# hsiehScalAR/KNODE-Cosserat

Measured on AMD Instinct MI355X. Metric: rod-steps/sec (N=100 segments, batch=1024), higher is better.
Workload: dtype f64

## Files before the change

knode-cosserat_amd/csrc/kr_mso_impl.hpp:

```cpp
#pragma once
#include "kr_ms_impl.hpp"

namespace kr {

constexpr int MSO_B0 = 7 + 17 * (MS_P - 1);
#ifndef KR_MSO_LAG
#define KR_MSO_LAG 1
#endif
constexpr int MSO_LAG = KR_MSO_LAG;
static_assert(MSO_B0 + MS_P <= WAVE, "the verifying lanes must fit beside the forward-difference lanes");

template <typename T, int HS>
__host__ __device__ inline size_t mso_lds_elems(int N) {
  return ms_lds_elems<T, HS>(N, true, false) + 80;
}

__device__ __forceinline__ void wave_sync_lds() {
  __builtin_amdgcn_fence(__ATOMIC_ACQ_REL, "wavefront");
  __builtin_amdgcn_wave_barrier();
}

#define KR_LDS __attribute__((address_space(3)))
template <typename T, int NV>
__device__ __forceinline__ void lds_load_vec(const T* src, T (&v)[NV]) {
  using V = typename Vec16<T>::type;
  constexpr int n = Vec16<T>::n;
  static_assert(NV % n == 0, "vector load needs a multiple of 16 bytes");
  const KR_LDS V* s = (const KR_LDS V*)src;
#pragma unroll
  for (int c = 0; c < NV / n; ++c) {
    const V x = s[c];
#pragma unroll
    for (int e = 0; e < n; ++e) v[c * n + e] = x[e];
  }
}
template <typename T, int NV>
__device__ __forceinline__ void lds_store_vec(T* dst, const T (&v)[NV]) {
  using V = typename Vec16<T>::type;
  constexpr int n = Vec16<T>::n;
  static_assert(NV % n == 0, "vector store needs a multiple of 16 bytes");
  KR_LDS V* d = (KR_LDS V*)dst;
#pragma unroll
  for (int c = 0; c < NV / n; ++c) {
    V x;
#pragma unroll
    for (int e = 0; e < n; ++e) x[e] = v[c * n + e];
    d[c] = x;
  }
}

#ifdef KR_MS_STAMPS
struct MsoStats { unsigned long long total = 0, sweeps = 0, merged = 0, quick = 0, chord = 0, rejects = 0, retries = 0, rebuilds = 0, t_sweep = 0, t_alg = 0, t_pred = 0, t_verdict = 0, t_cond = 0, t_fin = 0, t_upd = 0, t_v1 = 0, t_v2 = 0, t_c1 = 0, t_c2 = 0, t_copy = 0; };
#endif

template <typename T, bool DIAG, int HS, int OCC = 1, typename PSRC = RodConst<T>>
__global__ __launch_bounds__(WAVE * MS_WPB, OCC) void mso_sim_kernel(const PSRC Pa, const SimArgs<T> A) {
  extern __shared__ __attribute__((aligned(16))) unsigned char smem_raw[];
  const int N = rod_src_N<T>(Pa);
  const int lane = threadIdx.x & (WAVE - 1);
  const int wv = threadIdx.x / WAVE;
  const int64_t rod = (int64_t)blockIdx.x * MS_WPB + wv;
  if (rod >= A.B) return;
  const auto& Pc = rod_src_row<T>(Pa, rod);
  const size_t rod_elems = (size_t)N * KR_SLOTS;
  const int64_t T_steps = A.T_steps;
  const MsLds<T> L = ms_carve<T, HS>(reinterpret_cast<T*>(smem_raw) + (size_t)wv * mso_lds_elems<T, HS>(N), N, true, false);
  T* const Xs = L.Xs;
  T* const Es = L.Es;
  T* const XB = L.XB;
  T* const Tm = L.Tm;
  T* const XsB = L.c12 + (size_t)N * 12;
  T* const EsB = Es + MSO_B0 * MS_YP;
  const MsRole R = ms_role(lane, N);
  const int iv = R.iv, col = R.col;
  const bool isA = lane < MSO_B0;
  const bool isB = lane >= MSO_B0 && lane < MSO_B0 + MS_P;
  const int ib = isB ? lane - MSO_B0 : 0;
  const int s_l = isB ? ms_interval_start(ib, R.sbase, R.srem) : R.s_i;
  const int len_l = isB ? R.sbase + (ib < R.srem ? 1 : 0) : R.len_i;
  ms_cold_fill<T>(rod_src_mem<T>(Pa, rod), L.cold, lane);
  wave_sync();

  auto state_ptr = [&](int64_t k) -> T* { return A.states + (A.ring ? k % 3 : k) * A.slot_elems + rod * rod_elems; };
  T* const lead0 = L.c12;
  const ptrdiff_t lead_d = L.hist - L.c12;
  auto lead_of = [&](int64_t t) -> T* { return lead0 + (ptrdiff_t)(t & 1) * lead_d; };
  auto rebuild = [&](int64_t t) {
    const T* cur = state_ptr(t);
    const T* prv = t > 0 ? state_ptr(t - 1) : (A.prev_init ? A.prev_init + rod * rod_elems : cur);
    T* const lc = lead_of(t);
    T* const lp = lead_of(t - 1);
    for (int j = lane; j < N; j += WAVE) {
      T cv[12], pv[12];
      load_hist_vec<T, 12>(cur + (size_t)j * KR_SLOTS, cv);
      load_hist_vec<T, 12>(prv + (size_t)j * KR_SLOTS, pv);
      lds_store_vec<T, 12>(lc + (size_t)j * 12, cv);
      lds_store_vec<T, 12>(lp + (size_t)j * 12, pv);
    }
    wave_sync();
  };
  const T* ctl = A.ctl + rod * T_steps * 4;
  auto load_fc = [&](int64_t t) -> V3<T> {
    V3<T> tf{T(0), T(0), T(0)};
#pragma unroll
    for (int k = 0; k < 4; ++k) {
      const T tt = ctl[t * 4 + k];
      tf.x += tt * L.cold[CD_TDIRS + k * 3 + 0];
      tf.y += tt * L.cold[CD_TDIRS + k * 3 + 1];
      tf.z += tt * L.cold[CD_TDIRS + k * 3 + 2];
    }
    return {L.cold[CD_RHOAG] + tf.x, L.cold[CD_RHOAG + 1] + tf.y, L.cold[CD_RHOAG + 2] + tf.z};
  };

  const T* s0 = state_ptr(0);
  const T* sp0 = A.prev_init ? A.prev_init + rod * rod_elems : s0;
  MsPred<T> Q;
  double* img = A.pred_io ? A.pred_io + (size_t)rod * MS_PRED_ROWS * WAVE : nullptr;
  if (img && A.pred_load) ms_pred_load<T>(Q, img, lane);
  else ms_pred_init<T>(Q, lane, R, s0, sp0, A.prev_init != nullptr, A.predictor);
  V3<T> vlast, ulast;
  {
    const T* cl = s0 + (size_t)(N - 1) * KR_SLOTS;
    vlast = {cl[SL_V], cl[SL_V + 1], cl[SL_V + 2]};
    ulast = {cl[SL_U], cl[SL_U + 1], cl[SL_U + 2]};
  }
  const T tol = A.tol, tolA = A.tolA, fd_eps = A.fd_eps;
  const int maxit = A.maxit;
  T kappa = Q.kappa;
  T Gguess = lane < 6 ? A.G[rod * 6 + lane] : T(0);
  MsStamps stamps;
#ifdef KR_MS_STAMPS
  MsoStats st;
  unsigned long long t_begin, tq;
  KR_STAMP(t_begin);
  tq = t_begin;
#endif

  rebuild(0);

  int64_t tA = 0;
  bool merged = false;
  int it = 0;
  int order = Q.next_order;
  bool retried = false;
  T dn_prev = T(-1);
  bool have_fac = false, below = false;
  float amp = -1.f;
  T dnB = T(-1);
  float ampB = -1.f;
  bool belowB = false;
  int itB = 0, orderB = 0;
  bool pred_skip = false;
  bool reverify = false;
  int64_t resume_at = T_steps;
  T Xreg[MS_P - 1][2];
#pragma unroll
  for (int g = 0; g < MS_P - 1; ++g) Xreg[g][0] = Xreg[g][1] = T(0);
  const int kp = lane & 3;
  const int r = 3 + (lane >> 2);
  const bool plane = lane < 3 * (MS_P - 1);
  const int pi = plane ? lane / 3 : 0;
  const int prow = plane ? lane - 3 * pi : 0;
  const bool glane = lane >= WAVE - 6;
  V3<T> fcA = load_fc(0), fcB = fcA;
  V3<T> fcN = load_fc(T_steps > 1 ? 1 : 0);
  static_assert(DIAG, "the in-sweep history record assumes diagonal material matrices");
  T hk_a[3], hk_b[3], hk_c[3];
#pragma unroll
  for (int c = 0; c < 3; ++c) {
    hk_a[c] = L.cold[CD_KSEI + 4 * c] * L.cold[CD_KSEV + c];
    hk_b[c] = -L.cold[CD_KSEI + 4 * c] * L.cold[CD_BSE + 4 * c];
    hk_c[c] = -L.cold[CD_KBTI + 4 * c] * L.cold[CD_BBT + 4 * c];
  }

  ms_pred_guess<T>(Q, order, lane, L.cold, Xs);
  wave_sync_lds();
  if (order <= 0 && lane < 6) Xs[0 * MS_YP + 7 + lane] = Gguess;
  wave_sync_lds();

  struct Upd { T updP, updG, xsP, xsG, xsY[MS_P - 1]; };

  while (true) {
    const bool runA = tA < T_steps;
    const int64_t tB = tA - 1;
    T yr[19];
    {
      const T* src = isB ? XsB + ib * MS_YP : Xs + iv * MS_YP;
#pragma unroll
      for (int q = 0; q < 19; ++q) yr[q] = src[q];
    }
    const T hstep = (isA && col > 0) ? fd_eps * fmax(fabs(Xs[iv * MS_YP + (R.comp > 0 ? R.comp : 3)]), T(1)) : T(1);
#pragma unroll
    for (int q = 3; q < 19; ++q) yr[q] += (isA && q == R.comp) ? hstep : T(0);
    RodState<T> y = rows_to_state(yr);
    const V3<T> fc = isB ? fcB : fcA;
    const int lag = (isA && merged) ? MSO_LAG : 0;
    const bool act = isB ? merged : (isA && runA);
    const int trips = R.lmax + ((merged && runA) ? MSO_LAG : 0);
    T* const out_rod = state_ptr(tB + 1);
    auto point_of = [&](int k) -> int {
      const int kk = k - lag;
      return s_l + (kk < 0 ? 0 : (kk < len_l ? kk : len_l - 1));
    };
    const T* const lead_n = lead_of(isB ? tB : tA);
    const T* const lead_o = lead_of(isB ? tB + 1 : tB);
    auto hist_form = [&](const T (&la)[12], const T (&lb)[12]) __attribute__((always_inline)) -> RodHist<T> {
      T raw[12];
#pragma unroll
      for (int c = 0; c < 12; ++c) raw[c] = A.hc1 * la[c] + A.hc2 * lb[c];
      RodHist<T> h;
      h.qh = {raw[0], raw[1], raw[2]};
      h.wh = {raw[3], raw[4], raw[5]};
      h.vh = {raw[6], raw[7], raw[8]};
      h.uh = {raw[9], raw[10], raw[11]};
      h.av = {hk_b[0] * raw[6] + hk_a[0], hk_b[1] * raw[7] + hk_a[1], hk_b[2] * raw[8] + hk_a[2]};
      h.au = {hk_c[0] * raw[9], hk_c[1] * raw[10], hk_c[2] * raw[11]};
      return h;
    };
    auto hist_at = [&](int j) __attribute__((always_inline)) -> RodHist<T> {
      T la[12], lb[12];
      lds_load_vec<T, 12>(lead_n + (size_t)j * 12, la);
      lds_load_vec<T, 12>(lead_o + (size_t)j * 12, lb);
      return hist_form(la, lb);
    };
    RodHist<T> hst = hist_at(point_of(0));
    if (!merged) {
      auto fd_point = [&](int j, T dsl) __attribute__((always_inline)) {
        RodState<T> k1;
        V3<T> v, u;
        ode_eval<T, DIAG>(Pc, y, hst, fc, k1, v, u);
        hst = hist_at(j + 1);
        y = state_axpy(y, dsl, k1);
      };
#pragma unroll 2
      for (int t = 0; t < R.sbase; ++t) fd_point(R.s_i + t, Pc.ds);
      if (R.srem) fd_point(R.s_i + (R.len_i > R.sbase ? R.sbase : R.sbase - 1), R.len_i > R.sbase ? Pc.ds : T(0));
    } else {
      const bool lean = A.ring && tB + 4 <= T_steps;
      T* const lead_w = lead_of(tB + 1);
      auto trip = [&](int k, auto full_tag) __attribute__((always_inline)) {
        constexpr bool FULL = decltype(full_tag)::value;
        const int kk = k - lag;
        const bool live = FULL ? act : (act && kk >= 0 && kk < len_l);
        const int j = FULL ? s_l + kk : point_of(k);
        T la[12], lb[12];
        if constexpr (MSO_LAG >= 2) {
          const int jn = FULL ? j + 1 : point_of(k + 1);
          lds_load_vec<T, 12>(lead_n + (size_t)jn * 12, la);
          lds_load_vec<T, 12>(lead_o + (size_t)jn * 12, lb);
        }
        RodState<T> k1;
        V3<T> v, u;
        ode_eval<T, DIAG>(Pc, y, hst, fc, k1, v, u);
        if constexpr (MSO_LAG >= 2) {
          hst = hist_form(la, lb);
          asm volatile("" : "+v"(hst.qh.x), "+v"(hst.qh.y), "+v"(hst.qh.z), "+v"(hst.wh.x), "+v"(hst.wh.y), "+v"(hst.wh.z));
          asm volatile("" : "+v"(hst.vh.x), "+v"(hst.vh.y), "+v"(hst.vh.z), "+v"(hst.uh.x), "+v"(hst.uh.y), "+v"(hst.uh.z));
          asm volatile("" : "+v"(hst.av.x), "+v"(hst.av.y), "+v"(hst.av.z), "+v"(hst.au.x), "+v"(hst.au.y), "+v"(hst.au.z));
        }
        if (isB && live) {
          T rec[KR_SLOTS];
          record_from(y, v, u, rec);
          T lead[12];
#pragma unroll
          for (int c = 0; c < 12; ++c) lead[c] = rec[c];
          if constexpr (FULL) {
            if (!lean) {
              T rest[KR_SLOTS - 12];
#pragma unroll
              for (int c = 0; c < KR_SLOTS - 12; ++c) rest[c] = rec[12 + c];
              store_vec<T, KR_SLOTS - 12>(out_rod + (size_t)j * KR_SLOTS + 12, rest);
            }
          } else {
            store_record(out_rod + (size_t)j * KR_SLOTS, rec);
          }
          lds_store_vec<T, 12>(lead_w + (size_t)j * 12, lead);
        }
        if constexpr (MSO_LAG < 2) hst = hist_at(FULL ? j + 1 : point_of(k + 1));
        const T dsl = live ? Pc.ds : T(0);
        y = state_axpy(y, dsl, k1);
      };
      int k = 0;
      for (; k < MSO_LAG && k < trips; ++k) trip(k, std::false_type{});
#pragma unroll 2
      for (; k < R.sbase; ++k) trip(k, std::true_type{});
      for (; k < trips; ++k) trip(k, std::false_type{});
    }
#ifdef KR_MS_STAMPS
    KR_STAMP_ADD(st.t_sweep, tq);
    st.sweeps += 1;
    if (merged) st.merged += 1;
#endif

    T er[19];
    state_to_rows(y, er);
    T d[6];
    T updY[MS_P - 1];
    T* dYb = XB;
    float dnf = 0.f;
    bool finite = true;
    Upd U;

    auto finish = [&](const T* X, auto base_slot) -> float {
      T* sp = Tm;
      if (kp == 0) {
#pragma unroll
        for (int g = 1; g < MS_P - 1; ++g) dYb[g * MS_YP + r] = updY[g - 1];
      }
      wave_sync_lds();
      if (plane) {
        const int l0 = pi == 0 ? 0 : 7 + 17 * (pi - 1);
        T s = Es[base_slot(pi) * MS_YP + prow] - X[(pi + 1) * MS_YP + prow];
        T av[16], dv[16];
#pragma unroll
        for (int c = 0; c < 16; ++c) {
          const bool use = pi > 0 || c < 6;
          av[c] = use ? Es[(l0 + 1 + c) * MS_YP + prow] : T(0);
          dv[c] = pi > 0 ? dYb[pi * MS_YP + 3 + c] : T(0);
        }
        __builtin_amdgcn_sched_barrier(0);
        T s2 = T(0);
#pragma unroll
        for (int c = 0; c < 16; c += 2) {
          const T da = pi > 0 ? dv[c] : (c < 6 ? d[c < 6 ? c : 0] : T(0));
          const T db = pi > 0 ? dv[c + 1] : (c + 1 < 6 ? d[c + 1 < 6 ? c + 1 : 0] : T(0));
          s = fma(av[c], da, s);
          s2 = fma(av[c + 1], db, s2);
        }
        sp[pi * 3 + prow] = s + s2;
      }
      wave_sync_lds();
      float nf = 0.f;
      U.updP = T(0); U.updG = T(0); U.xsP = T(0); U.xsG = T(0);
      if (plane) {
        U.xsP = X[(pi + 1) * MS_YP + prow];
#pragma unroll
        for (int i = 0; i < MS_P - 1; ++i) {
          const T t = sp[i * 3 + prow];
          U.updP += i <= pi ? t : T(0);
        }
        nf = update_ratio(U.updP, U.xsP);
      }
      if (glane) {
        const int k = lane - (WAVE - 6);
        U.xsG = X[0 * MS_YP + 7 + k];
        U.updG = k == 0 ? d[0] : k == 1 ? d[1] : k == 2 ? d[2] : k == 3 ? d[3] : k == 4 ? d[4] : d[5];
        nf = fmaxf(nf, update_ratio(U.updG, U.xsG));
      }
#pragma unroll
      for (int g = 1; g < MS_P; ++g) {
        U.xsY[g - 1] = T(0);
        if (((g - 1) & 3) == kp) {
          U.xsY[g - 1] = X[g * MS_YP + r];
          nf = fmaxf(nf, update_ratio(updY[g - 1], U.xsY[g - 1]));
        }
      }
      return wave_max_nonneg(nf);
    };
    auto apply = [&](T* X) {
      if (plane) X[(pi + 1) * MS_YP + prow] = U.xsP + U.updP;
      if (glane) X[0 * MS_YP + 7 + (lane - (WAVE - 6))] = U.xsG + U.updG;
#pragma unroll
      for (int g = 1; g < MS_P; ++g)
        if (((g - 1) & 3) == kp) X[g * MS_YP + r] = U.xsY[g - 1] + updY[g - 1];
    };

    if (merged) {
      if (isB) {
#pragma unroll
        for (int q = 0; q < 19; ++q) EsB[ib * MS_YP + q] = er[q];
        if (ib == MS_P - 1) {
          T rec[KR_SLOTS];
          record_from(y, vlast, ulast, rec);
          store_record(out_rod + (size_t)(N - 1) * KR_SLOTS, rec);
          T lead[12];
#pragma unroll
          for (int c = 0; c < 12; ++c) lead[c] = rec[c];
          lds_store_vec<T, 12>(lead_of(tB + 1) + (size_t)(N - 1) * 12, lead);
          if (A.tip) {
            T* tp = A.tip + (rod * T_steps + tB) * 3;
            tp[0] = y.p.x; tp[1] = y.p.y; tp[2] = y.p.z;
          }
        }
      }
      wave_sync_lds();
#ifdef KR_MS_STAMPS
      unsigned long long tv;
      { KR_STAMP(tv); st.t_v1 += tv - tq; }
#endif
      float rn = 0.f;
      if (lane < 3 * MS_YP) {
        const int g = lane / MS_YP, q = lane - MS_YP * g;
        const T x = XsB[(g + 1) * MS_YP + q];
        rn = update_ratio(EsB[g * MS_YP + q] - x, x);
      } else if (lane < 3 * MS_YP + 6) {
        const int k = lane - 3 * MS_YP;
        const T e = EsB[(MS_P - 1) * MS_YP + 7 + k];
        rn = update_ratio(L.cold[CD_FTIP + k] - e, e);
      }
      rn = wave_max_nonneg(rn);
#ifdef KR_MS_STAMPS
      KR_STAMP_ADD(st.t_v2, tv);
#endif
      const float est = ampB * rn;
      bool accepted = A.residual_test != 0 && ampB > 0.f && T(256) * (T)est <= tol;
      float dnv = est;
#ifdef KR_MS_STAMPS
      if (accepted) st.quick += 1;
#endif
      if (!accepted) {
        T* ach = XB;
        T* rt = XB + 4 * MS_YP;
        dYb = XB + MS_YP * 8;
        T areg[MS_P - 1];
        areg[0] = EsB[0 * MS_YP + r] - XsB[1 * MS_YP + r];
        if (kp == 0) ach[1 * MS_YP + r] = areg[0];
        wave_sync_lds();
#pragma unroll
        for (int g = 1; g < MS_P; ++g) {
          const int l0 = 7 + 17 * (g - 1);
          T av[4], xv[4];
#pragma unroll
          for (int cc = 0; cc < 4; ++cc) {
            av[cc] = Es[(l0 + 1 + 4 * kp + cc) * MS_YP + r];
            xv[cc] = ach[g * MS_YP + 3 + 4 * kp + cc];
          }
          const T e0 = EsB[g * MS_YP + r];
          const T ynext = g < MS_P - 1 ? XsB[(g + 1) * MS_YP + r] : T(0);
          T part = fma(av[0], xv[0], av[1] * xv[1]) + fma(av[2], xv[2], av[3] * xv[3]);
          part += quad_xor<0xB1>(part);
          part += quad_xor<0x4E>(part);
          if (g < MS_P - 1) {
            areg[g] = e0 - ynext + part;
            if (kp == 0) ach[(g + 1) * MS_YP + r] = areg[g];
          } else if (kp == 0 && r >= 7 && r < 13) {
            rt[r - 7] = L.cold[CD_FTIP + (r - 7)] - e0 - part;
          }
          wave_sync_lds();
        }
        {
          T rtv[6];
#pragma unroll
          for (int j = 0; j < 6; ++j) rtv[j] = rt[j];
#pragma unroll
          for (int i = 0; i < 6; ++i) {
            T acc = T(0);
#pragma unroll
            for (int j = 0; j < 6; ++j) acc = fma(L.Ti[i * 6 + j], rtv[j], acc);
            d[i] = acc;
          }
        }
        {
          const T dd0 = kp == 0 ? T(0) : kp == 1 ? d[1] : kp == 2 ? d[3] : d[5];
          const T dd1 = kp == 0 ? d[0] : kp == 1 ? d[2] : kp == 2 ? d[4] : T(0);
#pragma unroll
          for (int g = 1; g < MS_P; ++g) {
            T sx = fma(Xreg[g - 1][1], dd1, Xreg[g - 1][0] * dd0);
            sx += quad_xor<0xB1>(sx);
            sx += quad_xor<0x4E>(sx);
            updY[g - 1] = areg[g - 1] + sx;
          }
        }
        dnv = finish(XsB, [](int g) { return MSO_B0 + g; });
        accepted = dnv <= 3.0e38f && (T)dnv <= T(0.5) * tol;
#ifdef KR_MS_STAMPS
        st.chord += 1;
#endif
      }
      if (accepted) {
        {
          const T* const lt = lead_of(tB + 1);
          for (int j = lane; j < N; j += WAVE) {
            T lv[12];
            lds_load_vec<T, 12>(lt + (size_t)j * 12, lv);
            store_vec<T, 12>(out_rod + (size_t)j * KR_SLOTS, lv);
          }
        }
        if (!belowB && dnB > T(0)) {
          const T floor_dn = T(64) * (sizeof(T) == 8 ? T(2.2e-16) : T(1.2e-7));
          const T kq = fmax((T)dnv, floor_dn) * fast_rcp(dnB * dnB);
          kappa = fmin(fmax(kq, T(1e-4)), T(1));
        }
        if (lane == 0 && A.status) A.status[rod * T_steps + tB] = KR_ST_CONVERGED;
        if (lane < 6) Gguess = XsB[0 * MS_YP + 7 + lane];
        pred_skip = false;
        reverify = false;
        merged = false;
        if (!runA) break;
      } else {
#ifdef KR_MS_STAMPS
        st.rejects += 1;
#endif
        const bool ok = dnv <= 3.0e38f;
        if (ok) apply(XsB);
        wave_sync_lds();
        if (ok && !reverify && itB + 2 <= maxit) {
          reverify = true;
          itB += 1;
          dnB = (T)dnv;
          __builtin_amdgcn_fence(__ATOMIC_ACQ_REL, "agent");
          rebuild(tB);
#ifdef KR_MS_STAMPS
          st.rebuilds += 1;
          KR_STAMP_ADD(st.t_alg, tq);
#endif
          continue;
        }
        reverify = false;
        for (int e = lane; e < MS_NE; e += WAVE) Xs[e] = XsB[e];
        tA = tB;
        fcN = fcA;
        fcA = fcB;
        order = orderB;
        it = itB;
        dn_prev = ok ? (T)dnv : T(-1);
        have_fac = ok;
        amp = ampB;
        below = false;
        pred_skip = true;
        merged = false;
        __builtin_amdgcn_fence(__ATOMIC_ACQ_REL, "agent");
        rebuild(tA);
#ifdef KR_MS_STAMPS
        st.rebuilds += 1;
        KR_STAMP_ADD(st.t_alg, tq);
#endif
        if (it >= maxit) { resume_at = tA; break; }
        continue;
      }
    }

#ifdef KR_MS_STAMPS
    { unsigned long long t_; KR_STAMP(t_); st.t_verdict += t_ - tq; }
    unsigned long long tq2;
    KR_STAMP(tq2);
#endif
    ++it;
    float res_full;
    {
      const int l0own = iv == 0 ? 0 : 7 + 17 * (iv - 1);
      if (isA && col == 0) {
#pragma unroll
        for (int q = 0; q < 19; ++q) Es[lane * MS_YP + q] = er[q];
      }
      wave_sync_lds();
      res_full = ms_residual_norm<T>(Es, Xs, L.cold, lane);
      if (isA && col > 0) {
        const T ih = fast_rcp(hstep);
        T e0[19];
#pragma unroll
        for (int q = 0; q < 19; ++q) e0[q] = Es[l0own * MS_YP + q];
        __builtin_amdgcn_sched_barrier(0);
#pragma unroll
        for (int q = 0; q < 19; ++q) Es[lane * MS_YP + q] = (er[q] - e0[q]) * ih;
      }
      wave_sync_lds();
    }
#ifdef KR_MS_STAMPS
    unsigned long long tc;
    { KR_STAMP(tc); st.t_c1 += tc - tq2; }
#endif
    dYb = XB;
    {
      const T c0 = Es[0 * MS_YP + r] - Xs[1 * MS_YP + r];
      const T da = Es[(2 * kp) * MS_YP + r];
      const T db = Es[(2 * kp + 1) * MS_YP + r];
      Xreg[0][0] = kp == 0 ? c0 : da;
      Xreg[0][1] = kp == 3 ? T(0) : db;
      store_pair(XB + r * 8 + 2 * kp, Xreg[0][0], Xreg[0][1]);
    }
    wave_sync_lds();
#pragma unroll
    for (int g = 1; g < MS_P; ++g) {
      const T* xcur = XB + ((g - 1) & 1) * (MS_YP * 8);
      T* xnext = XB + (g & 1) * (MS_YP * 8);
      const int l0 = 7 + 17 * (g - 1);
      const T e0 = Es[l0 * MS_YP + r];
      T n0 = T(0), n1 = T(0), n2 = T(0), n3 = T(0);
      if (g < MS_P - 1) {
        const T cg = e0 - Xs[(g + 1) * MS_YP + r];
        n0 = kp == 0 ? cg : T(0);
      }
      {
        T av[16], xa[16], xb[16];
#pragma unroll
        for (int c = 0; c < 16; ++c) {
          av[c] = Es[(l0 + 1 + c) * MS_YP + r];
          load_pair(xcur + (3 + c) * 8 + 2 * kp, xa[c], xb[c]);
        }
        __builtin_amdgcn_sched_barrier(0);
#pragma unroll
        for (int c = 0; c < 16; c += 2) {
          n0 = fma(av[c], xa[c], n0);
          n1 = fma(av[c], xb[c], n1);
          n2 = fma(av[c + 1], xa[c + 1], n2);
          n3 = fma(av[c + 1], xb[c + 1], n3);
        }
        n0 += n2;
        n1 += n3;
      }
      if (g < MS_P - 1) {
        Xreg[g][0] = n0;
        Xreg[g][1] = n1;
        store_pair(xnext + r * 8 + 2 * kp, n0, n1);
      } else if (r >= 7 && r < 13) {
        if (kp == 0) n0 = L.cold[CD_FTIP + (r - 7)] - e0 - n0;
        store_pair(Tm + (r - 7) * 8 + 2 * kp, n0, n1);
      }
      wave_sync_lds();
    }
#ifdef KR_MS_STAMPS
    KR_STAMP_ADD(st.t_c2, tc);
#endif
    {
      T a6[6][7];
#pragma unroll
      for (int i = 0; i < 6; ++i) {
        T row[8];
        load_hist_vec<T, 8>(Tm + i * 8, row);
#pragma unroll
        for (int k = 0; k < 6; ++k) a6[i][k] = row[1 + k];
        a6[i][6] = lane < 6 ? (lane == i ? T(1) : T(0)) : row[0];
      }
      T x6[6];
      solve6(a6, x6);
      if (lane < 6) {
#pragma unroll
        for (int i = 0; i < 6; ++i) L.Ti[i * 6 + lane] = x6[i];
      }
#pragma unroll
      for (int i = 0; i < 6; ++i) d[i] = lane_bcast<6>(x6[i]);
      have_fac = true;
    }
    {
      const T dd0 = kp == 0 ? T(1) : kp == 1 ? d[1] : kp == 2 ? d[3] : d[5];
      const T dd1 = kp == 0 ? d[0] : kp == 1 ? d[2] : kp == 2 ? d[4] : T(0);
#pragma unroll
      for (int g = 1; g < MS_P; ++g) {
        T s = fma(Xreg[g - 1][1], dd1, Xreg[g - 1][0] * dd0);
        s += quad_xor<0xB1>(s);
        s += quad_xor<0x4E>(s);
        updY[g - 1] = s;
      }
    }
#ifdef KR_MS_STAMPS
    KR_STAMP_ADD(st.t_cond, tq2);
#endif
    dnf = finish(Xs, [](int g) { return g == 0 ? 0 : 7 + 17 * (g - 1); });
#ifdef KR_MS_STAMPS
    KR_STAMP_ADD(st.t_fin, tq2);
#endif
    finite = dnf <= 3.0e38f;
    const T dn = (T)dnf;
    if (res_full > 0.f && finite) amp = dnf / res_full;
    if (finite && !below && dn <= tol) {
      below = true;
      if (dn_prev > T(0)) {
        const T floor_dn = T(64) * (sizeof(T) == 8 ? T(2.2e-16) : T(1.2e-7));
        const T kq = fmax(dn, floor_dn) * fast_rcp(dn_prev * dn_prev);
        kappa = fmin(fmax(kq, T(1e-4)), T(1));
      }
    }
    bool next_final = false;
    if (finite) {
      apply(Xs);
      next_final = predict_final<T>(dn, dn_prev, tol, tolA) || (kappa > T(0) && T(4) * kappa * dn * dn <= tol);
      dn_prev = dn;
    }
    wave_sync_lds();
#ifdef KR_MS_STAMPS
    KR_STAMP_ADD(st.t_alg, tq);
#endif
    if (!finite || (it >= maxit && !(next_final && dn <= T(1e-2)))) {
      if (order > 0 && !retried) {
        retried = true;
        order = 0;
        ms_pred_guess<T>(Q, 0, lane, L.cold, Xs);
        wave_sync_lds();
        if (lane < 6) Xs[0 * MS_YP + 7 + lane] = Gguess;
        wave_sync_lds();
        it = 0; dn_prev = T(-1); have_fac = false; amp = -1.f; below = false;
#ifdef KR_MS_STAMPS
        st.retries += 1;
#endif
        continue;
      }
      resume_at = tA;
      break;
    }
    if (next_final && dn <= T(1e-2)) {
      for (int e = lane; e < MS_NE; e += WAVE) XsB[e] = Xs[e];
      wave_sync_lds();
#ifdef KR_MS_STAMPS
      { unsigned long long t_; KR_STAMP(t_); st.t_copy += t_ - tq; }
#endif
      dnB = dn; ampB = amp; belowB = below; itB = it; orderB = order;
      if (!pred_skip) ms_pred_update<T>(Q, order, KR_ST_CONVERGED, A.predictor, lane, XsB, stamps);
#ifdef KR_MS_STAMPS
      { unsigned long long t_; KR_STAMP(t_); st.t_upd += t_ - tq; }
#endif
      tA += 1;
      fcB = fcA;
      if (tA < T_steps) {
        fcA = fcN;
        fcN = load_fc(tA + 1 < T_steps ? tA + 1 : tA);
        order = Q.next_order;
        ms_pred_guess<T>(Q, order, lane, L.cold, Xs);
        wave_sync_lds();
        if (order <= 0 && lane < 6) Xs[0 * MS_YP + 7 + lane] = XsB[0 * MS_YP + 7 + lane];
        wave_sync_lds();
      }
      it = 0; retried = false; below = false; dn_prev = T(-1);
      merged = true;
#ifdef KR_MS_STAMPS
      KR_STAMP_ADD(st.t_pred, tq);
#endif
    }
  }

  if (lane < 6) A.G[rod * 6 + lane] = Gguess;
  if (lane == 0 && A.resume) A.resume[rod] = (int32_t)resume_at;
  if (img && (resume_at >= T_steps || !A.resume)) {
    Q.kappa = kappa;
    ms_pred_save<T>(Q, img, lane);
  }
#ifdef KR_MS_STAMPS
  if (lane == 0 && A.dbg) {
    unsigned long long te;
    KR_STAMP(te);
    unsigned long long* dd = A.dbg + rod * 24;
    dd[0] = te - t_begin; dd[1] = st.t_sweep; dd[2] = st.t_alg; dd[3] = st.t_pred; dd[4] = st.sweeps;
    dd[5] = st.merged; dd[6] = st.quick; dd[7] = st.chord; dd[8] = st.rejects; dd[9] = st.retries; dd[10] = st.rebuilds;
    dd[11] = (unsigned long long)resume_at;
    dd[12] = st.t_verdict; dd[13] = st.t_cond; dd[14] = st.t_fin; dd[15] = st.t_upd;
    dd[16] = stamps.a1; dd[17] = stamps.a2; dd[18] = stamps.a3; dd[19] = st.t_v1; dd[20] = st.t_v2; dd[21] = st.t_c1; dd[22] = st.t_c2; dd[23] = st.t_copy;
  }
#endif
}

template <typename T>
int prepare_mso_sim(kr_handle* h, int64_t B) {
  const RodConst<T>& P = consts<T>(h);
  constexpr int HS = hs_phys<T>();
  if (!P.diag || P.N - 1 < 2 * MS_P) return 1;
  const size_t smem = sizeof(T) * mso_lds_elems<T, HS>(P.N) * MS_WPB;
  if (smem > (size_t)h->lds_limit) return 1;
  hipFuncAttributes fa;
  if (sizeof(T) == 4 && B > 1024 && 2 * smem <= (size_t)h->lds_limit) {
    auto k2 = mso_sim_kernel<T, true, HS, 2>;
    KR_HIP(hipFuncGetAttributes(&fa, reinterpret_cast<const void*>(k2)));
    if (int rc_lds_ = dyn_lds(reinterpret_cast<const void*>(k2), smem)) return rc_lds_;
  } else {
    auto k1 = mso_sim_kernel<T, true, HS, 1>;
    KR_HIP(hipFuncGetAttributes(&fa, reinterpret_cast<const void*>(k1)));
    if (int rc_lds_ = dyn_lds(reinterpret_cast<const void*>(k1), smem)) return rc_lds_;
  }
  return KR_OK;
}

template <typename T>
int launch_mso_sim(kr_handle* h, const SimArgs<T>& a, hipStream_t s) {
  const RodConst<T>& P = consts<T>(h);
  constexpr int HS = hs_phys<T>();
  if (!P.diag || P.N - 1 < 2 * MS_P) return 1;
  const size_t smem = sizeof(T) * mso_lds_elems<T, HS>(P.N) * MS_WPB;
  if (smem > (size_t)h->lds_limit) return 1;
  const dim3 grid((unsigned)((a.B + MS_WPB - 1) / MS_WPB)), block(WAVE * MS_WPB);
  if constexpr (sizeof(T) == 4) {
    if (a.B > 1024 && 2 * smem <= (size_t)h->lds_limit) {
      auto kern2 = mso_sim_kernel<T, true, HS, 2>;
      if (int rc_lds_ = dyn_lds(reinterpret_cast<const void*>(kern2), smem)) return rc_lds_;
      hipLaunchKernelGGL(kern2, grid, block, smem, s, P, a);
      KR_HIP(hipGetLastError());
      return KR_OK;
    }
  }
  auto kern = mso_sim_kernel<T, true, HS, 1>;
  if (int rc_lds_ = dyn_lds(reinterpret_cast<const void*>(kern), smem)) return rc_lds_;
  hipLaunchKernelGGL(kern, grid, block, smem, s, P, a);
  KR_HIP(hipGetLastError());
  return KR_OK;
}

}
```

knode-cosserat_amd/csrc/kr_sim_impl.hpp:

```cpp
#pragma once
#include "kr_internal.hpp"
#include "mlp_lane.hpp"
#include "mlp_mfma.hpp"
#include "mlp_jvp.hpp"

namespace kr {

constexpr int RPW = 8;
constexpr int WAVE = 64;

template <typename T>
struct Vec16;
template <>
struct Vec16<float> {
  typedef float type __attribute__((ext_vector_type(4)));
  static constexpr int n = 4;
};
template <>
struct Vec16<double> {
  typedef double type __attribute__((ext_vector_type(2)));
  static constexpr int n = 2;
};

template <typename T>
// ... 80 lines not shown
  constexpr int NR = (HS == HS_NNH) ? 25 : 12;
  constexpr int NRP = (NR + Vec16<T>::n - 1) / Vec16<T>::n * Vec16<T>::n;
  T cv[NRP], pv[NRP];
  load_hist_vec<T, NRP>(c, cv);
  load_hist_vec<T, NRP>(p, pv);
  T raw[NR];
#pragma unroll
  for (int k = 0; k < NR; ++k) raw[k] = hc1 * cv[k] + hc2 * pv[k];
#pragma unroll
  for (int k = 0; k < 12; ++k) hv[k] = raw[k];
  RodHist<T> h;
  h.qh = {raw[0], raw[1], raw[2]};
  h.wh = {raw[3], raw[4], raw[5]};
  h.vh = {raw[6], raw[7], raw[8]};
  h.uh = {raw[9], raw[10], raw[11]};
  hist_derive(P, h);
  hv[12] = h.av.x; hv[13] = h.av.y; hv[14] = h.av.z;
  hv[15] = h.au.x; hv[16] = h.au.y; hv[17] = h.au.z;
  if constexpr (HS == HS_NNH) {
#pragma unroll
    for (int k = 0; k < 13; ++k) hv[18 + k] = raw[12 + k];
    hv[31] = T(0);
  } else if constexpr (HS > 18) {
    hv[18] = T(0);
    hv[19] = T(0);
  }
}
template <typename T, int HS>
__device__ __forceinline__ void build_hist_point(const RodConst<T>& P, T hc1, T hc2, const T* __restrict__ c,
                                                 const T* __restrict__ p, T* dst) {
  T hv[HS];
  build_hist_vals<T, HS>(P, hc1, hc2, c, p, hv);
  using V = typename Vec16<T>::type;
  constexpr int n = Vec16<T>::n;
  V* d = reinterpret_cast<V*>(dst);
#pragma unroll
  for (int k = 0; k < HS / n; ++k) {
    V v;
#pragma unroll
    for (int e = 0; e < n; ++e) v[e] = hv[k * n + e];
    d[k] = v;
  }
}

template <typename T>
__device__ __forceinline__ bool predict_final(T dn, T dn_prev, T tol, T tolA) {
  if (dn <= tolA) return true;
  if (!(dn_prev > T(0)) || !(dn < dn_prev)) return false;
  T kappa = dn * fast_rcp(dn_prev * dn_prev);
  kappa = fmin(fmax(kappa, T(1e-3)), T(1));
  return T(4) * kappa * dn * dn <= tol;
}

template <typename T>
__device__ __forceinline__ void solve6(T (&a)[6][7], T (&x)[6]) {
  T inv[6];
#pragma unroll
  for (int k = 0; k < 6; ++k) {
#pragma unroll
    for (int i = k + 1; i < 6; ++i) {
      if (__builtin_expect(fabs(a[i][k]) > fabs(a[k][k]), 0)) {
#pragma unroll
        for (int c = k; c < 7; ++c) {
          const T t = a[k][c];
          a[k][c] = a[i][c];
          a[i][c] = t;
        }
      }
    }
    inv[k] = fast_rcp(a[k][k]);
#pragma unroll
    for (int i = k + 1; i < 6; ++i) {
      const T f = a[i][k] * inv[k];
#pragma unroll
      for (int c = k + 1; c < 7; ++c) a[i][c] = fma(-f, a[k][c], a[i][c]);
    }
  }
#pragma unroll
  for (int k = 5; k >= 0; --k) {
    T s = a[k][6];
#pragma unroll
    for (int c = k + 1; c < 6; ++c) s = fma(-a[k][c], x[c], s);
    x[k] = s * inv[k];
  }
}

struct NnRole {
  int iv = 0, col = 0;
  bool idle = false, jvp = false;
  int zrow = -1;
  int xrow = -1;
  int ptab = 0;
  bool lowp = false;
  bool base_only = false;
};
template <typename T, int HS, int VAR = 0, bool JVP_ONLY = false>
__device__ __forceinline__ void nn_correct(const MlpDev<T>& M, T* bufA, T* bufB, int stride, T* tile, int lane,
                                           const NnRole& role, const RodState<T>& y, const T (&hv)[HS], V3<T> tf,
                                           RodState<T>& ys, V3<T>& v, V3<T>& u) {
  T yr[19];
  state_to_rows(y, yr);
  if constexpr (HS != HS_NNH) {
    if (JVP_ONLY || M.mfma_ok) {
      T x[MM_IN];
#pragma unroll
      for (int i = 0; i < 19; ++i) x[i] = yr[i];
      x[19] = v.x; x[20] = v.y; x[21] = v.z; x[22] = u.x; x[23] = u.y; x[24] = u.z;
      x[25] = tf.x; x[26] = tf.y; x[27] = tf.z;
      T d[25];
      if constexpr (JVP_ONLY) {
        mlp_jvp_eval<T, VAR>(M, x, tile, lane, role.iv, role.col, role.idle, role.zrow, d, role.xrow, role.ptab, role.lowp, role.base_only);
      } else {
        if (role.jvp && M.jvp_ok) mlp_jvp_eval<T, VAR>(M, x, tile, lane, role.iv, role.col, role.idle, role.zrow, d, role.xrow, role.ptab, role.lowp, role.base_only);
        else mlp_mfma_eval<T>(M, x, tile, lane, d);
      }
      T yr2[19];
      state_to_rows(ys, yr2);
#pragma unroll
      for (int i = 0; i < 19; ++i) yr2[i] += d[i];
      ys = rows_to_state(yr2);
      v = {v.x + d[19], v.y + d[20], v.z + d[21]};
      u = {u.x + d[22], u.y + d[23], u.z + d[24]};
      return;
    }
  }
  int o = 0;
#pragma unroll
  for (int i = 0; i < 19; ++i) bufA[(o + i) * stride] = yr[i];
  o += 19;
  if constexpr (HS == HS_NNH) {
#pragma unroll
    for (int i = 0; i < 13; ++i) bufA[(o + i) * stride] = hv[18 + i];
#pragma unroll
    for (int i = 0; i < 6; ++i) bufA[(o + 13 + i) * stride] = hv[i];
    o += 19;
  }
  bufA[(o + 0) * stride] = v.x; bufA[(o + 1) * stride] = v.y; bufA[(o + 2) * stride] = v.z;
  bufA[(o + 3) * stride] = u.x; bufA[(o + 4) * stride] = u.y; bufA[(o + 5) * stride] = u.z;
  o += 6;
  if constexpr (HS == HS_NNH) {
#pragma unroll
    for (int i = 0; i < 6; ++i) bufA[(o + i) * stride] = hv[6 + i];
    o += 6;
  }
  bufA[(o + 0) * stride] = tf.x; bufA[(o + 1) * stride] = tf.y; bufA[(o + 2) * stride] = tf.z;
  const T* out = mlp_lane_eval<T>(M, bufA, bufB, stride);
  T d[25];
#pragma unroll
  for (int i = 0; i < 25; ++i) d[i] = out[i * stride];
  T yr2[19];
  state_to_rows(ys, yr2);
#pragma unroll
  for (int i = 0; i < 19; ++i) yr2[i] += d[i];
  ys = rows_to_state(yr2);
  v = {v.x + d[19], v.y + d[20], v.z + d[21]};
  u = {u.x + d[22], u.y + d[23], u.z + d[24]};
}

template <typename T, int HS>
struct SweepCtx {
  const T* hbase;
  T* bufA;
  T* bufB;
  int astride;
  T* tile;
  int lane;
// ... 517 lines not shown
```

knode-cosserat_amd/csrc/kr_tab_impl.hpp:

```cpp
#pragma once
#include "kr_mso_impl.hpp"

namespace kr {

template <typename T>
__global__ void init_straight_tab_kernel(int N, const double* __restrict__ Ls, int64_t B, T* __restrict__ state) {
  const int64_t pts = B * (int64_t)N;
  for (int64_t i = (int64_t)blockIdx.x * blockDim.x + threadIdx.x; i < pts; i += (int64_t)gridDim.x * blockDim.x) {
    const int j = (int)(i % N);
    const double L = Ls[i / N];
    T rec[KR_SLOTS];
#pragma unroll
    for (int k = 0; k < KR_SLOTS; ++k) rec[k] = T(0);
    rec[SL_P + 2] = (T)((double)j * (L / (double)(N - 1)));
    if (j == N - 1) rec[SL_P + 2] = (T)L;
    rec[SL_H] = T(1);
    rec[SL_V + 2] = T(1);
    store_record(state + i * KR_SLOTS, rec);
  }
}

template <typename T>
int launch_tab_init_straight(kr_handle* h, const kr_param_table* t, T* state, hipStream_t s) {
  hipLaunchKernelGGL((init_straight_tab_kernel<T>), dim3(grid_for(t->B * t->N)), dim3(256), 0, s, t->N, t->L, t->B, state);
  KR_HIP(hipGetLastError());
  return KR_OK;
}

static inline int tab_refuse(const std::string& why) {
  set_error("kr_simulate_batch_table: " + why + " (not served with a parameter table; nothing falls back to the handle's parameters)");
  return KR_E_UNSUPPORTED;
}

template <typename T>
int launch_tab_sim(kr_handle* h, const kr_param_table* t, int scheme, int use_nn, const SimArgs<T>& a, hipStream_t s) {
  constexpr int HS = hs_phys<T>();
  const int N = t->N;
  if (scheme != KR_EULER) return tab_refuse("only Euler sweeps (scheme = KR_EULER)");
  if (N - 1 < 2 * MS_P || N > MS_NPL * WAVE) return tab_refuse("N = " + std::to_string(N) + ", the one-wavefront persistent kernels serve 9 <= N <= 128");
  if (h->ms_mode == 0 || h->persistent == 0) return tab_refuse("options ms_mode = 0 / persistent = 0 select kernels without a table form");
  if (h->ms_mode != 1 && a.B > (int64_t)h->ms_batch_limit) return tab_refuse("B exceeds option ms_batch_limit");
  if (h->waves_per_rod > 1) return tab_refuse("option waves_per_rod = " + std::to_string(h->waves_per_rod) + ", table calls run one wavefront per rod");
  if (a.B > (int64_t)0x7fffffff) return tab_refuse("B >= 2^31");
  const MlpDev<T>& M = mlpdev<T>(h);
  if (use_nn) {
    if (M.n_layers <= 0) { set_error("use_nn requested but no MLP was set (kr_set_mlp)"); return KR_E_STATE; }
    if (!M.mfma_ok || !M.jvp_ok || h->params.nn_input_history) return tab_refuse("an MLP the persistent one-wavefront kernel does not evaluate");
  }
  const RodTable<T> tab{(const KR_CONSTANT_AS RodConst<T>*)table_rows<T>(t), N};
  const dim3 grid((unsigned)((a.B + MS_WPB - 1) / MS_WPB)), block(WAVE * MS_WPB);
  h->last_waves_per_rod = 1;
  h->last_overlap = 0;
  if (use_nn) {
    const size_t smem = ms_lds_bytes<T, HS>(N, true, true);
    if (smem > (size_t)h->lds_limit) return tab_refuse("the rod's history does not fit the LDS with the MLP on");
    auto kern = ms_sim_kernel<T, true, KR_EULER, HS, true, 1, RodTable<T>>;
    if (int rc = dyn_lds(reinterpret_cast<const void*>(kern), smem)) return rc;
    hipLaunchKernelGGL(kern, grid, block, smem, s, tab, a, M);
    KR_HIP(hipGetLastError());
    return KR_OK;
  }
  const size_t smem = ms_lds_bytes<T, HS>(N, true);
  if (smem > (size_t)h->lds_limit) return tab_refuse("the rod's history does not fit the LDS");
  SimArgs<T> a2 = a;
  const size_t smem_o = sizeof(T) * mso_lds_elems<T, HS>(N) * MS_WPB;
  if (h->overlap && smem_o <= (size_t)h->lds_limit) {
    if (int rc = ensure_resume(h, a.B)) return rc;
    a2.resume = static_cast<int32_t*>(h->resume_buf);
    auto ko = mso_sim_kernel<T, true, HS, 1, RodTable<T>>;
    if (int rc = dyn_lds(reinterpret_cast<const void*>(ko), smem_o)) return rc;
    hipLaunchKernelGGL(ko, grid, block, smem_o, s, tab, a2);
    KR_HIP(hipGetLastError());
    h->last_overlap = 1;
  }
  auto kern = ms_sim_kernel<T, true, KR_EULER, HS, false, 1, RodTable<T>>;
  if (int rc = dyn_lds(reinterpret_cast<const void*>(kern), smem)) return rc;
  hipLaunchKernelGGL(kern, grid, block, smem, s, tab, a2, M);
  KR_HIP(hipGetLastError());
  return KR_OK;
}

}
```

Baseline: 42.03 million.

## Pin uniform args in SGPRs, double-buffer Xs, use 32-bit step counters, pivot-free solve

Kernel arguments are forced into scalar registers with empty inline asm. Step counters become 32-bit, and the ring slot index is tracked incrementally instead of computed with a modulo each step. The copy of Xs into XsB on acceptance is replaced by swapping two buffer pointers. The 6x6 solve now runs without pivoting and only reloads and falls back to the pivoted version when any lane would have needed a row swap. These changes aim to reduce VGPR pressure, 64-bit arithmetic and LDS copies, and they add a T_steps < 2^31 check.

```diff
diff --git a/knode-cosserat_amd/csrc/kr_mso_impl.hpp b/knode-cosserat_amd/csrc/kr_mso_impl.hpp
--- a/knode-cosserat_amd/csrc/kr_mso_impl.hpp
+++ b/knode-cosserat_amd/csrc/kr_mso_impl.hpp
@@ -47,6 +47,19 @@
     for (int e = 0; e < n; ++e) x[e] = v[c * n + e];
     d[c] = x;
   }
+}
+
+template <typename U>
+__device__ __forceinline__ U own_sgpr(U v) {
+  asm volatile("" : "+s"(v));
+  return v;
+}
+
+template <typename U>
+__device__ __forceinline__ U* own_sgpr_global(U* p) {
+  uintptr_t v = (uintptr_t)p;
+  asm volatile("" : "+s"(v));
+  return (U*)(__attribute__((address_space(1))) U*)v;
 }
 
 #ifdef KR_MS_STAMPS
@@ -63,13 +76,23 @@
   if (rod >= A.B) return;
   const auto& Pc = rod_src_row<T>(Pa, rod);
   const size_t rod_elems = (size_t)N * KR_SLOTS;
-  const int64_t T_steps = A.T_steps;
+  T* const a_states = own_sgpr_global(A.states);
+  const int64_t a_slot_elems = own_sgpr(A.slot_elems);
+  const int a_ring = own_sgpr(A.ring);
+  T* const a_tip = own_sgpr_global(A.tip);
+  int32_t* const a_status = own_sgpr_global(A.status);
+  const int a_residual_test = own_sgpr(A.residual_test), a_predictor = own_sgpr(A.predictor);
+  const T hc1 = own_sgpr(A.hc1), hc2 = own_sgpr(A.hc2);
+  const int T_steps = own_sgpr((int)A.T_steps);
   const MsLds<T> L = ms_carve<T, HS>(reinterpret_cast<T*>(smem_raw) + (size_t)wv * mso_lds_elems<T, HS>(N), N, true, false);
-  T* const Xs = L.Xs;
   T* const Es = L.Es;
   T* const XB = L.XB;
   T* const Tm = L.Tm;
-  T* const XsB = L.c12 + (size_t)N * 12;
+  T* const X0 = L.Xs;
+  const ptrdiff_t X_d = (L.c12 + (size_t)N * 12) - L.Xs;
+  int xsel = 0;
+  T* Xs = X0;
+  T* XsB = X0 + X_d;
   T* const EsB = Es + MSO_B0 * MS_YP;
   const MsRole R = ms_role(lane, N);
   const int iv = R.iv, col = R.col;
@@ -81,11 +104,12 @@
   ms_cold_fill<T>(rod_src_mem<T>(Pa, rod), L.cold, lane);
   wave_sync();
 
-  auto state_ptr = [&](int64_t k) -> T* { return A.states + (A.ring ? k % 3 : k) * A.slot_elems + rod * rod_elems; };
+  auto slot_ptr = [&](int slot) -> T* { return a_states + (int64_t)slot * a_slot_elems + rod * rod_elems; };
+  auto state_ptr = [&](int k) -> T* { return slot_ptr(a_ring ? k % 3 : k); };
   T* const lead0 = L.c12;
   const ptrdiff_t lead_d = L.hist - L.c12;
-  auto lead_of = [&](int64_t t) -> T* { return lead0 + (ptrdiff_t)(t & 1) * lead_d; };
-  auto rebuild = [&](int64_t t) {
+  auto lead_of = [&](int t) -> T* { return lead0 + (ptrdiff_t)(t & 1) * lead_d; };
+  auto rebuild = [&](int t) {
     const T* cur = state_ptr(t);
     const T* prv = t > 0 ? state_ptr(t - 1) : (A.prev_init ? A.prev_init + rod * rod_elems : cur);
     T* const lc = lead_of(t);
@@ -99,12 +123,12 @@
     }
     wave_sync();
   };
-  const T* ctl = A.ctl + rod * T_steps * 4;
-  auto load_fc = [&](int64_t t) -> V3<T> {
+  const T* ctl = A.ctl + rod * A.T_steps * 4;
+  auto load_fc = [&](int t) -> V3<T> {
     V3<T> tf{T(0), T(0), T(0)};
 #pragma unroll
     for (int k = 0; k < 4; ++k) {
-      const T tt = ctl[t * 4 + k];
+      const T tt = ctl[(size_t)t * 4 + k];
       tf.x += tt * L.cold[CD_TDIRS + k * 3 + 0];
       tf.y += tt * L.cold[CD_TDIRS + k * 3 + 1];
       tf.z += tt * L.cold[CD_TDIRS + k * 3 + 2];
@@ -117,15 +141,15 @@
   MsPred<T> Q;
   double* img = A.pred_io ? A.pred_io + (size_t)rod * MS_PRED_ROWS * WAVE : nullptr;
   if (img && A.pred_load) ms_pred_load<T>(Q, img, lane);
-  else ms_pred_init<T>(Q, lane, R, s0, sp0, A.prev_init != nullptr, A.predictor);
+  else ms_pred_init<T>(Q, lane, R, s0, sp0, A.prev_init != nullptr, a_predictor);
   V3<T> vlast, ulast;
   {
     const T* cl = s0 + (size_t)(N - 1) * KR_SLOTS;
     vlast = {cl[SL_V], cl[SL_V + 1], cl[SL_V + 2]};
     ulast = {cl[SL_U], cl[SL_U + 1], cl[SL_U + 2]};
   }
-  const T tol = A.tol, tolA = A.tolA, fd_eps = A.fd_eps;
-  const int maxit = A.maxit;
+  const T tol = own_sgpr(A.tol), tolA = own_sgpr(A.tolA), fd_eps = own_sgpr(A.fd_eps);
+  const int maxit = own_sgpr(A.maxit);
   T kappa = Q.kappa;
   T Gguess = lane < 6 ? A.G[rod * 6 + lane] : T(0);
   MsStamps stamps;
@@ -138,7 +162,8 @@
 
   rebuild(0);
 
-  int64_t tA = 0;
+  int tA = 0;
+  int rsA = 0;
   bool merged = false;
   int it = 0;
   int order = Q.next_order;
@@ -152,16 +177,10 @@
   int itB = 0, orderB = 0;
   bool pred_skip = false;
   bool reverify = false;
-  int64_t resume_at = T_steps;
+  int resume_at = T_steps;
   T Xreg[MS_P - 1][2];
 #pragma unroll
   for (int g = 0; g < MS_P - 1; ++g) Xreg[g][0] = Xreg[g][1] = T(0);
-  const int kp = lane & 3;
-  const int r = 3 + (lane >> 2);
-  const bool plane = lane < 3 * (MS_P - 1);
-  const int pi = plane ? lane / 3 : 0;
-  const int prow = plane ? lane - 3 * pi : 0;
-  const bool glane = lane >= WAVE - 6;
   V3<T> fcA = load_fc(0), fcB = fcA;
   V3<T> fcN = load_fc(T_steps > 1 ? 1 : 0);
   static_assert(DIAG, "the in-sweep history record assumes diagonal material matrices");
@@ -182,7 +201,7 @@
 
   while (true) {
     const bool runA = tA < T_steps;
-    const int64_t tB = tA - 1;
+    const int tB = tA - 1;
     T yr[19];
     {
       const T* src = isB ? XsB + ib * MS_YP : Xs + iv * MS_YP;
@@ -190,14 +209,16 @@
       for (int q = 0; q < 19; ++q) yr[q] = src[q];
     }
     const T hstep = (isA && col > 0) ? fd_eps * fmax(fabs(Xs[iv * MS_YP + (R.comp > 0 ? R.comp : 3)]), T(1)) : T(1);
-#pragma unroll
-    for (int q = 3; q < 19; ++q) yr[q] += (isA && q == R.comp) ? hstep : T(0);
+    int comp = R.comp;
+    asm volatile("" : "+v"(comp));
+#pragma unroll
+    for (int q = 3; q < 19; ++q) yr[q] += q == comp ? hstep : T(0);
     RodState<T> y = rows_to_state(yr);
     const V3<T> fc = isB ? fcB : fcA;
     const int lag = (isA && merged) ? MSO_LAG : 0;
     const bool act = isB ? merged : (isA && runA);
     const int trips = R.lmax + ((merged && runA) ? MSO_LAG : 0);
-    T* const out_rod = state_ptr(tB + 1);
+    T* const out_rod = slot_ptr(rsA);
     auto point_of = [&](int k) -> int {
       const int kk = k - lag;
       return s_l + (kk < 0 ? 0 : (kk < len_l ? kk : len_l - 1));
@@ -207,7 +228,7 @@
     auto hist_form = [&](const T (&la)[12], const T (&lb)[12]) __attribute__((always_inline)) -> RodHist<T> {
       T raw[12];
 #pragma unroll
-      for (int c = 0; c < 12; ++c) raw[c] = A.hc1 * la[c] + A.hc2 * lb[c];
+      for (int c = 0; c < 12; ++c) raw[c] = hc1 * la[c] + hc2 * lb[c];
       RodHist<T> h;
       h.qh = {raw[0], raw[1], raw[2]};
       h.wh = {raw[3], raw[4], raw[5]};
@@ -236,7 +257,7 @@
       for (int t = 0; t < R.sbase; ++t) fd_point(R.s_i + t, Pc.ds);
       if (R.srem) fd_point(R.s_i + (R.len_i > R.sbase ? R.sbase : R.sbase - 1), R.len_i > R.sbase ? Pc.ds : T(0));
     } else {
-      const bool lean = A.ring && tB + 4 <= T_steps;
+      const bool lean = a_ring && tB + 4 <= T_steps;
       T* const lead_w = lead_of(tB + 1);
       auto trip = [&](int k, auto full_tag) __attribute__((always_inline)) {
         constexpr bool FULL = decltype(full_tag)::value;
@@ -292,6 +313,14 @@
     if (merged) st.merged += 1;
 #endif
 
+    int ln = lane;
+    asm volatile("" : "+v"(ln));
+    const int kp = ln & 3;
+    const int r = 3 + (ln >> 2);
+    const bool plane = ln < 3 * (MS_P - 1);
+    const int pi = plane ? ln / 3 : 0;
+    const int prow = plane ? ln - 3 * pi : 0;
+    const bool glane = ln >= WAVE - 6;
     T er[19];
     state_to_rows(y, er);
     T d[6];
@@ -342,7 +371,7 @@
         nf = update_ratio(U.updP, U.xsP);
       }
       if (glane) {
-        const int k = lane - (WAVE - 6);
+        const int k = ln - (WAVE - 6);
         U.xsG = X[0 * MS_YP + 7 + k];
         U.updG = k == 0 ? d[0] : k == 1 ? d[1] : k == 2 ? d[2] : k == 3 ? d[3] : k == 4 ? d[4] : d[5];
         nf = fmaxf(nf, update_ratio(U.updG, U.xsG));
@@ -359,7 +388,7 @@
     };
     auto apply = [&](T* X) {
       if (plane) X[(pi + 1) * MS_YP + prow] = U.xsP + U.updP;
-      if (glane) X[0 * MS_YP + 7 + (lane - (WAVE - 6))] = U.xsG + U.updG;
+      if (glane) X[0 * MS_YP + 7 + (ln - (WAVE - 6))] = U.xsG + U.updG;
 #pragma unroll
       for (int g = 1; g < MS_P; ++g)
         if (((g - 1) & 3) == kp) X[g * MS_YP + r] = U.xsY[g - 1] + updY[g - 1];
@@ -377,8 +406,8 @@
 #pragma unroll
           for (int c = 0; c < 12; ++c) lead[c] = rec[c];
           lds_store_vec<T, 12>(lead_of(tB + 1) + (size_t)(N - 1) * 12, lead);
-          if (A.tip) {
-            T* tp = A.tip + (rod * T_steps + tB) * 3;
+          if (a_tip) {
+            T* tp = a_tip + (rod * T_steps + tB) * 3;
             tp[0] = y.p.x; tp[1] = y.p.y; tp[2] = y.p.z;
           }
         }
@@ -389,12 +418,12 @@
       { KR_STAMP(tv); st.t_v1 += tv - tq; }
 #endif
       float rn = 0.f;
-      if (lane < 3 * MS_YP) {
-        const int g = lane / MS_YP, q = lane - MS_YP * g;
+      if (ln < 3 * MS_YP) {
+        const int g = ln / MS_YP, q = ln - MS_YP * g;
         const T x = XsB[(g + 1) * MS_YP + q];
         rn = update_ratio(EsB[g * MS_YP + q] - x, x);
-      } else if (lane < 3 * MS_YP + 6) {
-        const int k = lane - 3 * MS_YP;
+      } else if (ln < 3 * MS_YP + 6) {
+        const int k = ln - 3 * MS_YP;
         const T e = EsB[(MS_P - 1) * MS_YP + 7 + k];
         rn = update_ratio(L.cold[CD_FTIP + k] - e, e);
       }
@@ -403,7 +432,7 @@
       KR_STAMP_ADD(st.t_v2, tv);
 #endif
       const float est = ampB * rn;
-      bool accepted = A.residual_test != 0 && ampB > 0.f && T(256) * (T)est <= tol;
+      bool accepted = a_residual_test != 0 && ampB > 0.f && T(256) * (T)est <= tol;
       float dnv = est;
 #ifdef KR_MS_STAMPS
       if (accepted) st.quick += 1;
@@ -470,7 +499,7 @@
       if (accepted) {
         {
           const T* const lt = lead_of(tB + 1);
-          for (int j = lane; j < N; j += WAVE) {
+          for (int j = ln; j < N; j += WAVE) {
             T lv[12];
             lds_load_vec<T, 12>(lt + (size_t)j * 12, lv);
             store_vec<T, 12>(out_rod + (size_t)j * KR_SLOTS, lv);
@@ -481,8 +510,8 @@
           const T kq = fmax((T)dnv, floor_dn) * fast_rcp(dnB * dnB);
           kappa = fmin(fmax(kq, T(1e-4)), T(1));
         }
-        if (lane == 0 && A.status) A.status[rod * T_steps + tB] = KR_ST_CONVERGED;
-        if (lane < 6) Gguess = XsB[0 * MS_YP + 7 + lane];
+        if (ln == 0 && a_status) a_status[rod * T_steps + tB] = KR_ST_CONVERGED;
+        if (ln < 6) Gguess = XsB[0 * MS_YP + 7 + ln];
         pred_skip = false;
         reverify = false;
         merged = false;
@@ -507,8 +536,9 @@
           continue;
         }
         reverify = false;
-        for (int e = lane; e < MS_NE; e += WAVE) Xs[e] = XsB[e];
+        for (int e = ln; e < MS_NE; e += WAVE) Xs[e] = XsB[e];
         tA = tB;
+        rsA = a_ring ? (rsA == 0 ? 2 : rsA - 1) : rsA - 1;
         fcN = fcA;
         fcA = fcB;
         order = orderB;
@@ -541,10 +571,10 @@
       const int l0own = iv == 0 ? 0 : 7 + 17 * (iv - 1);
       if (isA && col == 0) {
 #pragma unroll
-        for (int q = 0; q < 19; ++q) Es[lane * MS_YP + q] = er[q];
+        for (int q = 0; q < 19; ++q) Es[ln * MS_YP + q] = er[q];
       }
       wave_sync_lds();
-      res_full = ms_residual_norm<T>(Es, Xs, L.cold, lane);
+      res_full = ms_residual_norm<T>(Es, Xs, L.cold, ln);
       if (isA && col > 0) {
         const T ih = fast_rcp(hstep);
         T e0[19];
@@ -552,7 +582,7 @@
         for (int q = 0; q < 19; ++q) e0[q] = Es[l0own * MS_YP + q];
         __builtin_amdgcn_sched_barrier(0);
 #pragma unroll
-        for (int q = 0; q < 19; ++q) Es[lane * MS_YP + q] = (er[q] - e0[q]) * ih;
+        for (int q = 0; q < 19; ++q) Es[ln * MS_YP + q] = (er[q] - e0[q]) * ih;
       }
       wave_sync_lds();
     }
@@ -614,19 +644,22 @@
 #endif
     {
       T a6[6][7];
-#pragma unroll
-      for (int i = 0; i < 6; ++i) {
-        T row[8];
-        load_hist_vec<T, 8>(Tm + i * 8, row);
-#pragma unroll
-        for (int k = 0; k < 6; ++k) a6[i][k] = row[1 + k];
-        a6[i][6] = lane < 6 ? (lane == i ? T(1) : T(0)) : row[0];
-      }
+      auto fill6 = [&](T (&m)[6][7]) {
+#pragma unroll
+        for (int i = 0; i < 6; ++i) {
+          T row[8];
+          load_hist_vec<T, 8>(Tm + i * 8, row);
+#pragma unroll
+          for (int k = 0; k < 6; ++k) m[i][k] = row[1 + k];
+          m[i][6] = ln < 6 ? (ln == i ? T(1) : T(0)) : row[0];
+        }
+      };
+      fill6(a6);
       T x6[6];
-      solve6(a6, x6);
-      if (lane < 6) {
-#pragma unroll
-        for (int i = 0; i < 6; ++i) L.Ti[i * 6 + lane] = x6[i];
+      solve6_uniform(a6, x6, fill6);
+      if (ln < 6) {
+#pragma unroll
+        for (int i = 0; i < 6; ++i) L.Ti[i * 6 + ln] = x6[i];
       }
 #pragma unroll
       for (int i = 0; i < 6; ++i) d[i] = lane_bcast<6>(x6[i]);
@@ -675,9 +708,9 @@
       if (order > 0 && !retried) {
         retried = true;
         order = 0;
-        ms_pred_guess<T>(Q, 0, lane, L.cold, Xs);
+        ms_pred_guess<T>(Q, 0, ln, L.cold, Xs);
         wave_sync_lds();
-        if (lane < 6) Xs[0 * MS_YP + 7 + lane] = Gguess;
+        if (ln < 6) Xs[0 * MS_YP + 7 + ln] = Gguess;
         wave_sync_lds();
         it = 0; dn_prev = T(-1); have_fac = false; amp = -1.f; below = false;
 #ifdef KR_MS_STAMPS
@@ -689,17 +722,19 @@
       break;
     }
     if (next_final && dn <= T(1e-2)) {
-      for (int e = lane; e < MS_NE; e += WAVE) XsB[e] = Xs[e];
-      wave_sync_lds();
+      xsel ^= 1;
+      Xs = X0 + xsel * X_d;
+      XsB = X0 + (1 - xsel) * X_d;
 #ifdef KR_MS_STAMPS
       { unsigned long long t_; KR_STAMP(t_); st.t_copy += t_ - tq; }
 #endif
       dnB = dn; ampB = amp; belowB = below; itB = it; orderB = order;
-      if (!pred_skip) ms_pred_update<T>(Q, order, KR_ST_CONVERGED, A.predictor, lane, XsB, stamps);
+      if (!pred_skip) ms_pred_update<T>(Q, order, KR_ST_CONVERGED, a_predictor, lane, XsB, stamps);
 #ifdef KR_MS_STAMPS
       { unsigned long long t_; KR_STAMP(t_); st.t_upd += t_ - tq; }
 #endif
       tA += 1;
+      rsA = a_ring ? (rsA == 2 ? 0 : rsA + 1) : rsA + 1;
       fcB = fcA;
       if (tA < T_steps) {
         fcA = fcN;
@@ -736,6 +771,14 @@
     dd[16] = stamps.a1; dd[17] = stamps.a2; dd[18] = stamps.a3; dd[19] = st.t_v1; dd[20] = st.t_v2; dd[21] = st.t_c1; dd[22] = st.t_c2; dd[23] = st.t_copy;
   }
 #endif
+}
+
+inline int mso_check_steps(int64_t T_steps) {
+  if (T_steps > (int64_t)0x7fffffff) {
+    set_error("T_steps = " + std::to_string(T_steps) + ": the overlapped persistent kernel counts steps in 32 bits (T_steps < 2^31)");
+    return KR_E_ARG;
+  }
+  return KR_OK;
 }
 
 template <typename T>
@@ -765,6 +808,7 @@
   if (!P.diag || P.N - 1 < 2 * MS_P) return 1;
   const size_t smem = sizeof(T) * mso_lds_elems<T, HS>(P.N) * MS_WPB;
   if (smem > (size_t)h->lds_limit) return 1;
+  if (int rc_steps_ = mso_check_steps(a.T_steps)) return rc_steps_;
   const dim3 grid((unsigned)((a.B + MS_WPB - 1) / MS_WPB)), block(WAVE * MS_WPB);
   if constexpr (sizeof(T) == 4) {
     if (a.B > 1024 && 2 * smem <= (size_t)h->lds_limit) {
diff --git a/knode-cosserat_amd/csrc/kr_sim_impl.hpp b/knode-cosserat_amd/csrc/kr_sim_impl.hpp
--- a/knode-cosserat_amd/csrc/kr_sim_impl.hpp
+++ b/knode-cosserat_amd/csrc/kr_sim_impl.hpp
@@ -186,6 +186,35 @@
 #pragma unroll
     for (int c = k + 1; c < 6; ++c) s = fma(-a[k][c], x[c], s);
     x[k] = s * inv[k];
+  }
+}
+
+template <typename T, typename F>
+__device__ __forceinline__ void solve6_uniform(T (&a)[6][7], T (&x)[6], F&& reload) {
+  T inv[6];
+  bool moves = false;
+#pragma unroll
+  for (int k = 0; k < 6; ++k) {
+#pragma unroll
+    for (int i = k + 1; i < 6; ++i) moves = moves | (fabs(a[i][k]) > fabs(a[k][k]));
+    inv[k] = fast_rcp(a[k][k]);
+#pragma unroll
+    for (int i = k + 1; i < 6; ++i) {
+      const T f = a[i][k] * inv[k];
+#pragma unroll
+      for (int c = k + 1; c < 7; ++c) a[i][c] = fma(-f, a[k][c], a[i][c]);
+    }
+  }
+#pragma unroll
+  for (int k = 5; k >= 0; --k) {
+    T s = a[k][6];
+#pragma unroll
+    for (int c = k + 1; c < 6; ++c) s = fma(-a[k][c], x[c], s);
+    x[k] = s * inv[k];
+  }
+  if (__builtin_expect(__builtin_amdgcn_ballot_w64(moves) != 0, 0)) {
+    reload(a);
+    solve6(a, x);
   }
 }
 
diff --git a/knode-cosserat_amd/csrc/kr_tab_impl.hpp b/knode-cosserat_amd/csrc/kr_tab_impl.hpp
--- a/knode-cosserat_amd/csrc/kr_tab_impl.hpp
+++ b/knode-cosserat_amd/csrc/kr_tab_impl.hpp
@@ -67,6 +67,7 @@
   if (h->overlap && smem_o <= (size_t)h->lds_limit) {
     if (int rc = ensure_resume(h, a.B)) return rc;
     a2.resume = static_cast<int32_t*>(h->resume_buf);
+    if (int rc = mso_check_steps(a.T_steps)) return rc;
     auto ko = mso_sim_kernel<T, true, HS, 1, RodTable<T>>;
     if (int rc = dyn_lds(reinterpret_cast<const void*>(ko), smem_o)) return rc;
     hipLaunchKernelGGL(ko, grid, block, smem_o, s, tab, a2);
```

Result: faster. 43.87 million, median of 6 (+4.4%).
